# yc-huang/bsdb

Measured on AMD Instinct MI355X. Metric: index-build keys/s (device-resident), 13B x 13-byte keys; % HBM roofline, higher is better.
Workload: dtype u64

## Files before the change

### bsdb_amd/csrc/bsdb_capi.hip

```cpp
#include <hip/hip_runtime.h>

#include <dlfcn.h>
#include <sched.h>
#include <fcntl.h>
#include <sys/mman.h>
#include <sys/stat.h>
#include <unistd.h>

#include <algorithm>
#include <atomic>
#include <cerrno>
#include <functional>
#include <chrono>
#include <condition_variable>
#include <cmath>
#include <cstdio>
#include <cstdlib>
#include <cstring>
#include <memory>
#include <mutex>
#include <new>
#include <shared_mutex>
#include <string>
#include <thread>
#include <condition_variable>
#include <deque>
#include <vector>

#include "../../include/bsdb_mi355x.h"
#include "hash_kernels.hip"
#include "fused_kernels.hip"
#include "mph_kernels.hip"
#include "gov_kernels.hip"
#include "verify_kernels.hip"

using namespace bsdb;

struct FeedSlot {
    void *buf[8] = {};
    size_t cap[8] = {};
    hipEvent_t copied = nullptr, done = nullptr;
    bool used = false;
    std::vector<uint64_t> reb;
};

struct bsdb_ctx {
    int device = 0;
    hipStream_t stream = nullptr;
    int hist_mode = 0;
    int frontend = 0;
    int num_cus = 256;
    int d13_variant = 13;
    int d13_copies = 8;
    uint64_t chunk_keys = 0;
    uint64_t span_max = 0;
    int fused = -1;
    int pipe = -1;
    uint64_t pipe_chunks = 0;
    uint32_t pipe_cus = 0;
    hipStream_t p2_stream = nullptr;
    hipEvent_t pipe_ev[6] = {};
    void *fu_ring = nullptr;
    size_t fu_ring_bytes = 0;
    uint64_t fu_launches = 0;
    std::mutex mu;
    void *ids = nullptr;
    size_t ids_bytes = 0;
    uint32_t *cursor = nullptr;
    size_t cursor_bytes = 0;
    uint64_t *p2_pref = nullptr;
    size_t p2_pref_bytes = 0;
    uint32_t *overflow = nullptr;
    uint64_t *scan_part = nullptr;
    size_t scan_part_n = 0;
    FeedSlot feed[2];
    hipStream_t copy_stream = nullptr;
    void *d_out = nullptr;
    size_t d_out_bytes = 0;
    void *g_sorted = nullptr, *g_counts = nullptr, *g_cursor = nullptr, *g_scratch = nullptr, *g_status = nullptr;
    size_t g_sorted_bytes = 0, g_counts_bytes = 0, g_cursor_bytes = 0, g_scratch_bytes = 0, g_status_bytes = 0;
    void *g_big = nullptr, *g_slabs = nullptr;
    size_t g_big_bytes = 0, g_slabs_bytes = 0;
    void *g_pay = nullptr;
    size_t g_pay_bytes = 0;
    void *g_led = nullptr;
    size_t g_led_bytes = 0;
    void *g_mid = nullptr;
    size_t g_mid_bytes = 0;
    void *g_midscr = nullptr;
    size_t g_midscr_bytes = 0;
    hipStream_t big_stream = nullptr;
    hipEvent_t big_ev[2] = {nullptr, nullptr};
    bool verify = false;
    hipEvent_t last_ev = nullptr;
    hipStream_t last_stream = nullptr;
    void *comm = nullptr;
    int nranks = 1, rank = 0;
    std::mutex mph_mu;
    std::vector<bsdb_mph *> mphs;
    void *pack = nullptr;
    size_t pack_bytes = 0;
    bool profiling = false;
    struct Rec { hipEvent_t a, b; int kind; uint64_t keys; };
    std::vector<Rec> recs;
    std::vector<hipEvent_t> pool;
    hipEvent_t ev() {
        if (!pool.empty()) { hipEvent_t e = pool.back(); pool.pop_back(); return e; }
        hipEvent_t e = nullptr;
        (void)hipEventCreate(&e);
        return e;
    }
};

struct Ordered {
    bsdb_ctx *c;
    hipStream_t s;
    Ordered(bsdb_ctx *c_, hipStream_t s_) : c(c_), s(s_) {
        if (c->last_ev && c->last_stream != s) (void)hipStreamWaitEvent(s, c->last_ev, 0);
    }
    ~Ordered() {
        if (!c->last_ev && hipEventCreateWithFlags(&c->last_ev, hipEventDisableTiming) != hipSuccess) c->last_ev = nullptr;
        if (c->last_ev) (void)hipEventRecord(c->last_ev, s);
        c->last_stream = s;
    }
};

struct ProfScope {
    bsdb_ctx *c; hipStream_t s; int kind; uint64_t keys; hipEvent_t a = nullptr;
    ProfScope(bsdb_ctx *c_, hipStream_t s_, int k, uint64_t n) : c(c_), s(s_), kind(k), keys(n) {
        if (c->profiling) { a = c->ev(); (void)hipEventRecord(a, s); }
    }
    ~ProfScope() {
        if (!a) return;
        hipEvent_t b = c->ev();
        (void)hipEventRecord(b, s);
        c->recs.push_back({a, b, kind, keys});
    }
};

static void comm_destroy(bsdb_ctx *c);

namespace {

constexpr uint64_t DEFAULT_CHUNK_KEYS = 1ULL << 32;
constexpr uint64_t MAX_SPAN_LAUNCHES = 8;

int hip_fail(hipError_t e, const char *what, int line) {
    static const bool dbg = getenv("BSDB_DEBUG") != nullptr;
    if (dbg) fprintf(stderr, "[bsdb] line %d: %s -> %d (%s)\n", line, what, (int)e, hipGetErrorString(e));
    return BSDB_EIO;
}
#define HIP_OK(x)                                                   \
    do {                                                            \
        const hipError_t e_ = (x);                                  \
        if (e_ != hipSuccess) return hip_fail(e_, #x, __LINE__);    \
    } while (0)

template <class T>
hipError_t dmalloc(T **p, size_t bytes) {
    const hipError_t e = hipMalloc(reinterpret_cast<void **>(p), bytes);
    if (e != hipSuccess) {
        (void)hipGetLastError();
        *p = nullptr;
    }
    return e;
}

int grow(void **p, size_t *have, size_t need) {
    if (*have >= need) return BSDB_OK;
    if (*p) (void)hipFree(*p);
    *p = nullptr;
    *have = 0;
    const size_t roomy = need >= (1u << 20) ? need + need / 64 : need;
    if (roomy != need && dmalloc(p, roomy) == hipSuccess) {
        *have = roomy;
        return BSDB_OK;
    }
    if (dmalloc(p, need) != hipSuccess) return BSDB_ENOMEM;
    *have = need;
    return BSDB_OK;
}

constexpr size_t XFER_PIECE = 32ull << 20;

struct PinnedPool {
    std::mutex mu;
    std::vector<void *> free_list;
    void *take() {
        {
            std::lock_guard<std::mutex> g(mu);
            if (!free_list.empty()) {
                void *p = free_list.back();
                free_list.pop_back();
                return p;
            }
        }
        void *p = nullptr;
        if (hipHostMalloc(&p, XFER_PIECE, hipHostMallocDefault) == hipSuccess) return p;
        (void)hipGetLastError();
        return nullptr;
    }
    void give(void *p) {
        if (!p) return;
        std::lock_guard<std::mutex> g(mu);
        free_list.push_back(p);
    }
};
PinnedPool &pinned_pool() {
    static PinnedPool *pool = new PinnedPool();
    return *pool;
}

int file_reserve(int fd, uint64_t off, uint64_t len) {
    if (fd < 0 || !len) return 0;
    int r;
    do {
        r = fallocate(fd, 0, (off_t)off, (off_t)len);
    } while (r != 0 && errno == EINTR);
    if (r == 0) return 0;
    return errno == EOPNOTSUPP || errno == ENOSYS ? 1 : -1;
}

struct Populator {
    std::thread th;
    std::atomic<bool> stop{false};
    std::atomic<uint64_t> ready{0};
    int fd = -1;
    uint64_t file_off = 0;
    double seconds = 0;
    Populator() = default;
    Populator(const Populator &) = delete;
    Populator &operator=(const Populator &) = delete;
    ~Populator() { finish(); }
    void start(uint8_t *base, uint64_t bytes, int file_fd = -1, uint64_t base_off = 0) {
        fd = file_fd;
        file_off = base_off;
        if (!base || !bytes || getenv("BSDB_NO_PREFAULT")) return;
        th = std::thread([this, base, bytes] {
            const auto t0 = std::chrono::steady_clock::now();
            constexpr uint64_t STEP = 16ull << 20;
            constexpr int MADV_POPULATE_WRITE_ = 23;
            bool madv = true;
            for (uint64_t o = 0; o < bytes && !stop.load(std::memory_order_relaxed); o += STEP) {
                const uint64_t k = std::min(STEP, bytes - o);
                if (fd >= 0) {
                    if (file_reserve(fd, file_off + o, k) != 0) break;
                    ready.store(o + k, std::memory_order_release);
                }
                if (madv) {
                    if (madvise(base + o, k, MADV_POPULATE_WRITE_) == 0) continue;
                    if (errno != EINVAL) break;
                    madv = false;
                }
                for (uint64_t q = 0; q < k; q += 4096) (void)*(volatile const uint8_t *)(base + o + q);
            }
            seconds = std::chrono::duration<double>(std::chrono::steady_clock::now() - t0).count();
        });
    }
    bool ensure(uint64_t off, uint64_t len) {
        if (fd < 0 || off + len <= ready.load(std::memory_order_acquire)) return true;
        return file_reserve(fd, file_off + off, len) == 0;
    }
    void finish() {
        stop.store(true);
        if (th.joinable()) th.join();
    }
};

int copy_on_own_stream(int dev, void *dst, const void *src, size_t bytes, hipMemcpyKind kind) {
    if (bytes == 0) return BSDB_OK;
    hipStream_t s = nullptr;
    hipError_t e = hipSetDevice(dev);
    if (e == hipSuccess) e = hipStreamCreateWithFlags(&s, hipStreamNonBlocking);
    if (e == hipSuccess) e = hipMemcpyAsync(dst, src, bytes, kind, s);
    if (e == hipSuccess) e = hipStreamSynchronize(s);
    if (s) (void)hipStreamDestroy(s);
    return e == hipSuccess ? BSDB_OK : hip_fail(e, kind == hipMemcpyHostToDevice ? "H2D copy (own stream)" : "D2H copy (own stream)", __LINE__);
}
struct BounceSlots {
    std::mutex mu;
    std::condition_variable cv;
    int free_slots;
    BounceSlots() {
        const char *e = getenv("BSDB_BOUNCE_SLOTS");
        const int v = e ? atoi(e) : 16;
        free_slots = v > 0 ? v : 1;
    }
    void acquire() {
        std::unique_lock<std::mutex> g(mu);
        cv.wait(g, [this] { return free_slots > 0; });
        --free_slots;
    }
    void release() {
        {
            std::lock_guard<std::mutex> g(mu);
            ++free_slots;
        }
        cv.notify_one();
    }
};
static BounceSlots &bounce_slots() {
    static BounceSlots *b = new BounceSlots();
    return *b;
}
int h2d_bounce(hipStream_t s, void *dst, const void *src, size_t bytes) {
    if (bytes == 0) return BSDB_OK;
    bounce_slots().acquire();
    void *pin[2] = {pinned_pool().take(), pinned_pool().take()};
    if (!pin[0] || !pin[1]) {
        pinned_pool().give(pin[0]);
        pinned_pool().give(pin[1]);
        bounce_slots().release();
        hipError_t e = hipMemcpyAsync(dst, src, bytes, hipMemcpyHostToDevice, s);
        if (e == hipSuccess) e = hipStreamSynchronize(s);
        return e == hipSuccess ? BSDB_OK : hip_fail(e, "H2D copy (pageable fallback)", __LINE__);
    }
    hipEvent_t ev[2] = {nullptr, nullptr};
    int rc = BSDB_OK;
    for (int i = 0; i < 2 && !rc; ++i)
        if (hipEventCreateWithFlags(&ev[i], hipEventDisableTiming) != hipSuccess) rc = BSDB_EIO;
    bool pending[2] = {false, false};
    for (size_t o = 0, k = 0; o < bytes && !rc; o += XFER_PIECE, ++k) {
        const int i = (int)(k & 1);
        const size_t len = std::min(XFER_PIECE, bytes - o);
        if (pending[i] && hipEventSynchronize(ev[i]) != hipSuccess) rc = BSDB_EIO;
        if (rc) break;
        memcpy(pin[i], (const uint8_t *)src + o, len);
        if (hipMemcpyAsync((uint8_t *)dst + o, pin[i], len, hipMemcpyHostToDevice, s) != hipSuccess ||
            hipEventRecord(ev[i], s) != hipSuccess)
            rc = BSDB_EIO;
        pending[i] = true;
    }
    if (hipStreamSynchronize(s) != hipSuccess && !rc) rc = BSDB_EIO;
    for (int i = 0; i < 2; ++i) {
        pinned_pool().give(pin[i]);
        if (ev[i]) (void)hipEventDestroy(ev[i]);
    }
    bounce_slots().release();
    return rc;
}

int d2h_pageable(int dev, void *dst, const void *src, size_t bytes) {
    return copy_on_own_stream(dev, dst, src, bytes, hipMemcpyDeviceToHost);
}
int h2d_pageable(int dev, void *dst, const void *src, size_t bytes) {
    return copy_on_own_stream(dev, dst, src, bytes, hipMemcpyHostToDevice);
}

hipStream_t pick(bsdb_ctx *, void *stream) { return (hipStream_t)stream; }

int launch_status() {
    const hipError_t e = hipGetLastError();
    return e == hipSuccess ? BSDB_OK : hip_fail(e, "kernel launch", 0);
}

int usable_cpus() {
    static const int n = [] {
        int c = (int)std::max(1u, std::thread::hardware_concurrency());
        cpu_set_t cs;
        if (sched_getaffinity(0, sizeof(cs), &cs) == 0) c = std::max(1, CPU_COUNT(&cs));
        if (FILE *f = fopen("/sys/fs/cgroup/cpu.max", "r")) {
            char q[32] = {0};
            unsigned long long per = 0;
            if (fscanf(f, "%31s %llu", q, &per) == 2 && strcmp(q, "max") != 0 && per > 0) {
                const unsigned long long quota = strtoull(q, nullptr, 10);
                if (quota > 0) c = std::min<int>(c, (int)std::max<unsigned long long>(1, (quota + per - 1) / per));
            }
            fclose(f);
        }
        return c;
    }();
    return n;
}

constexpr uint64_t MAX_TILES_PER_LAUNCH = (1ULL << 32) / P1_THREADS - 1;

template <int EPI>
void launch_pass1(const P1Args &a0, bool var, uint32_t key_len, uint64_t tiles, hipStream_t s, int frontend) {
    if (tiles > MAX_TILES_PER_LAUNCH) {
        for (uint64_t t0 = 0; t0 < tiles; t0 += MAX_TILES_PER_LAUNCH) {
            const uint64_t nt = std::min(MAX_TILES_PER_LAUNCH, tiles - t0);
            P1Args a = a0;
            const uint64_t k0 = t0 * P1_TILE;
            a.n = std::min<uint64_t>(a0.n - k0, nt * P1_TILE);
            if (var) {
                a.offsets = a0.offsets + k0;
            } else {
                a.keys = a0.keys + k0 * key_len;
                a.blob_bytes = a0.blob_bytes - k0 * key_len;
            }
            if (a.sig) a.sig = a0.sig + 2 * k0;
            launch_pass1<EPI>(a, var, key_len, nt, s, frontend);
        }
        return;
    }
    const P1Args &a = a0;
    const dim3 g((uint32_t)tiles), b(P1_THREADS);
    if (var && frontend == 2) {
        k_pass1<SRC_VAR, EPI, 1, 0><<<g, b, 0, s>>>(a);
    } else if (var) {
        k_pass1<SRC_VARSTAGED, EPI, 1, 0><<<g, b, 0, s>>>(a);
    } else if (key_len == 13 && frontend != 1) {
        k_pass1<SRC_DIRECT13, EPI, 4, 13><<<g, b, 0, s>>>(a);
    } else if (key_len == 13) {
        k_pass1<SRC_STAGED13, EPI, 4, 13><<<g, b, 0, s>>>(a);
    } else if (key_len >= 1 && key_len <= 13) {
        k_pass1<SRC_STAGED, EPI, 4, 0><<<g, b, 0, s>>>(a);
    } else if (key_len >= 14 && key_len <= 26) {
        k_pass1<SRC_STAGED, EPI, 2, 0><<<g, b, 0, s>>>(a);
    } else if (key_len >= 27 && key_len <= 52) {
        k_pass1<SRC_STAGED, EPI, 1, 0><<<g, b, 0, s>>>(a);
    } else {
        k_pass1<SRC_FIXED_DIRECT, EPI, 1, 0><<<g, b, 0, s>>>(a);
    }
}

struct PartPlan {
    uint32_t nparts;
    uint32_t bin_shift;
    uint32_t capb;
    uint32_t nmain;
    uint32_t ntail;
    uint32_t grid_d13;
    uint64_t cap;
    uint64_t cap_tail;
    size_t ids_elems() const { return (size_t)nparts * (nmain * cap + ntail * cap_tail); }
};

uint64_t round64(double x) { return ((uint64_t)x + 63) & ~63ULL; }

using D13Kernel = void (*)(P1Args, uint64_t);

struct Pass1Sel {
    D13Kernel k;
    int nt;
    uint64_t tile;
    bool binned;
    bool windowed;
    uint32_t bin_shift;
    uint32_t nparts;
    uint32_t capb;
};

bool binned_layout(Pass1Sel &sel, uint32_t maxp, uint32_t bin_ids, uint64_t m) {
    uint32_t shift = 0;
    while (shift <= (uint32_t)PART_SHIFT && ((m + (1ULL << shift) - 1) >> shift) > (uint64_t)maxp) ++shift;
    if (shift > (uint32_t)PART_SHIFT) return false;
    sel.bin_shift = shift;
    sel.nparts = (uint32_t)((m + (1ULL << shift) - 1) >> shift);
    sel.capb = std::min<uint32_t>((bin_ids / sel.nparts) & ~7u, (uint32_t)sel.tile + 8);
    return true;
}

Pass1Sel pass1_select(const bsdb_ctx *c, bool var, uint32_t key_len, bool seed0, uint64_t m) {
    const uint32_t nparts = (uint32_t)((m + PART_BUCKETS - 1) / PART_BUCKETS);
    const Pass1Sel none{nullptr, 0, 0, false, false, (uint32_t)PART_SHIFT, nparts, 0};
    const Pass1Sel sort{k_pass1_d13<512>, 512, 512 * P1_KEYS_PER_THREAD, false, true, (uint32_t)PART_SHIFT, nparts, 0};
    const bool sort_fits = nparts <= 1024;
    if (c->frontend != 0) return none;
    const bool k13 = !var && key_len == 13;
    const bool window = k13 || (!var && (key_len == 8 || key_len == 12 || key_len == 16) && !getenv("BSDB_NO_FIXED_WINDOW"));
    if (window) {
        if (k13 && c->d13_variant == 2) return sort_fits ? sort : none;
        D13Kernel k = key_len == 8    ? (seed0 ? k_pass1_d13e<0, true, 8> : k_pass1_d13e<0, false, 8>)
                      : key_len == 12 ? (seed0 ? k_pass1_d13e<0, true, 12> : k_pass1_d13e<0, false, 12>)
                      : key_len == 16 ? (seed0 ? k_pass1_d13e<0, true, 16> : k_pass1_d13e<0, false, 16>)
                      : c->d13_variant == 13 ? (seed0 ? k_pass1_d13e<13, true> : k_pass1_d13e<13>)
                                             : (seed0 ? k_pass1_d13e<0, true> : k_pass1_d13e<0>);
        Pass1Sel sel{k, D13E_NT, D13E_TILE, true, true, 0, 0, 0};
        if (binned_layout(sel, D13E_MAXP, D13E_BIN_IDS, m)) return sel;
        return k13 && sort_fits ? sort : none;
    }
    if (!var && (key_len == 0 || key_len > 32)) return none;
    D13Kernel k = var ? (seed0 ? k_pass1_vare<false, true> : k_pass1_vare<false>)
                      : (seed0 ? k_pass1_vare<true, true> : k_pass1_vare<true>);
    Pass1Sel sel{k, VARE_NT, VARE_TILE, true, false, 0, 0, 0};
    return binned_layout(sel, VARE_MAXP, VARE_BIN_IDS, m) ? sel : none;
}

PartPlan plan_partitions(const bsdb_ctx *c, uint64_t chunk, uint64_t m, const Pass1Sel &sel) {
    PartPlan p{};
    const bool d13 = sel.k != nullptr, binned = sel.binned;
    p.bin_shift = sel.bin_shift;
    p.nparts = sel.nparts;
    p.capb = sel.capb;
    const double frac = std::min(1.0, (double)(1ULL << p.bin_shift) / (double)m);
    p.nmain = binned ? (uint32_t)c->d13_copies : NCOPY;
    const double e = (double)chunk * frac / p.nmain;
    p.cap = round64(e * 1.02 + 8.0 * std::sqrt(e) + 2 * P1_TILE + 64);
    p.ntail = 0;
    p.cap_tail = 0;
    if (d13) {
        int per_cu = 0;
        if (hipOccupancyMaxActiveBlocksPerMultiprocessor(&per_cu, sel.k, sel.nt, 0) != hipSuccess || per_cu < 1) per_cu = 1;
        per_cu = std::min(per_cu, 2048 / sel.nt);
        const uint64_t tiles = (chunk + sel.tile - 1) / sel.tile;
        p.grid_d13 = (uint32_t)std::min<uint64_t>(tiles, (uint64_t)c->num_cus * per_cu);
        if (const char *v = getenv("BSDB_D13_GRID")) p.grid_d13 = (uint32_t)std::max<int64_t>(1, std::min<int64_t>(p.grid_d13, atoll(v)));
        if (binned) {
            const double tiles_per_copy = (double)tiles / p.nmain + 1;
            p.cap = round64(e * 1.02 + 8.0 * std::sqrt(e) + 7.0 * tiles_per_copy + 2 * P1_TILE + 64);
        }
        p.ntail = NCOPY;
        p.cap_tail = round64(std::max<uint64_t>(P1_TILE, sel.tile) + 64);
    }
    return p;
}

constexpr uint64_t FU_MIN_SUPER = 4;

int fused13_impl(bsdb_ctx *c, const uint8_t *keys, uint64_t blob_bytes, uint64_t n, uint64_t seed, uint64_t m,
                 uint32_t *counts, hipStream_t s, uint64_t *done) {
    *done = 0;
    const uint64_t per = (uint64_t)FU_OWNERS * FU_TILE;
    if (c->num_cus != FU_OWNERS || m == 0 || m > (uint64_t)FU_OWNERS * (FU_TCAP - 2)) return BSDB_OK;
    if (blob_bytes < 3) return BSDB_OK;
    const uint64_t nsuper = std::min(n / per, (blob_bytes - 3) / 13 / per);
    if (nsuper < FU_MIN_SUPER) return BSDB_OK;
    if (n / m > 16384) return BSDB_OK;
    static int per_cu = -1;
    if (per_cu < 0 && hipOccupancyMaxActiveBlocksPerMultiprocessor(&per_cu, k_hist13_fused<true>, FU_NT, 0) != hipSuccess)
        per_cu = 0;
    if (per_cu < 1) return BSDB_OK;
    const size_t sync_bytes = FU_SYNC_U64 * sizeof(uint64_t);
    const size_t ring_bytes = (size_t)FU_SLOTS * FU_SLOT_BYTES;
    int rc = grow(&c->fu_ring, &c->fu_ring_bytes, ring_bytes + sync_bytes);
    if (rc) return rc;
    FusedArgs fa{};
    fa.keys = keys;
    fa.nsuper = nsuper;
    fa.seed = seed;
    fa.mult = (uint32_t)(2 * m);
    fa.m = (uint32_t)m;
    fa.ring = (uint8_t *)c->fu_ring;
    fa.sync = (uint64_t *)((uint8_t *)c->fu_ring + ring_bytes);
    fa.overflow = c->overflow;
    fa.counts = counts;
    HIP_OK(hipMemsetAsync(fa.sync, 0, sync_bytes, s));
    HIP_OK(hipMemsetAsync(c->overflow, 0, sizeof(uint32_t), s));
    ++c->fu_launches;
    {
        ProfScope ps(c, s, 0, nsuper * per);
        if (seed == 0 && !getenv("BSDB_NO_SEED0"))
            k_hist13_fused<true><<<FU_OWNERS, FU_NT, 0, s>>>(fa);
        else
            k_hist13_fused<false><<<FU_OWNERS, FU_NT, 0, s>>>(fa);
    }
    P1Args af{};
    af.keys = keys;
    af.blob_bytes = blob_bytes;
    af.key_len = 13;
    af.n = nsuper * per;
    af.seed = seed;
    af.multiplier = 2 * m;
    af.counts = counts;
    af.overflow = c->overflow;
    k_overflow_fallback<SRC_FIXED_DIRECT, 0><<<1024, P1_THREADS, 0, s>>>(af);
    if ((rc = launch_status())) return rc;
    *done = nsuper * per;
    return BSDB_OK;
}

bool pipe_wanted(const bsdb_ctx *c) { return c->pipe == 1; }

uint32_t pipe_p2_cus(const bsdb_ctx *c) {
    const uint32_t k = c->pipe_cus ? c->pipe_cus : (uint32_t)c->num_cus / 8;
    return std::max<uint32_t>(1, std::min<uint32_t>(k, (uint32_t)c->num_cus / 2));
}

bool fused_wanted(const bsdb_ctx *c) {
    if (c->hist_mode == 3) return true;
    if (c->hist_mode != 0) return false;
    if (c->fused >= 0) return c->fused == 1;
    return false;
}

int histogram_impl(bsdb_ctx *c, const uint8_t *keys, const uint64_t *offsets, uint64_t blob_bytes,
                   uint32_t key_len, uint64_t n, uint64_t seed, uint64_t m, uint32_t *counts,
                   hipStream_t s) {
    if (n == 0) return BSDB_OK;
    const bool var = offsets != nullptr;
    if (!var && key_len == 13 && fused_wanted(c)) {
        uint64_t done = 0;
        const int rc = fused13_impl(c, keys, blob_bytes, n, seed, m, counts, s, &done);
        if (rc) return rc;
        if (done) return histogram_impl(c, keys + done * 13, nullptr, blob_bytes - done * 13, 13, n - done, seed, m,
                                        counts, s);
    }
    P1Args a{};
    a.keys = keys;
    a.offsets = offsets;
    a.blob_bytes = blob_bytes;
    a.key_len = key_len;
    a.seed = seed;
    a.multiplier = 2 * m;
    a.counts = counts;
    const uint32_t nparts = (uint32_t)((m + PART_BUCKETS - 1) / PART_BUCKETS);
    const bool atomic_mode = c->hist_mode == 2 || nparts > (uint32_t)MAX_PARTS;
    if (atomic_mode) {
        a.n = n;
        ProfScope ps(c, s, 0, n);
        launch_pass1<EPI_ATOMIC>(a, var, key_len, (n + P1_TILE - 1) / P1_TILE, s, c->frontend);
        return launch_status();
    }
    uint64_t chunk = c->chunk_keys ? c->chunk_keys : DEFAULT_CHUNK_KEYS;
    chunk = std::max<uint64_t>(P1_TILE, chunk / P1_TILE * P1_TILE);
    chunk = std::min<uint64_t>(chunk, (n + P1_TILE - 1) / P1_TILE * P1_TILE);
    const Pass1Sel sel = pass1_select(c, var, key_len, seed == 0 && !getenv("BSDB_NO_SEED0"), m);
    const bool d13 = sel.k != nullptr;
    const bool pipe_pl = pipe_wanted(c) && sel.windowed && sel.binned;
    if (pipe_pl && !c->chunk_keys) {
        const uint64_t nch = c->pipe_chunks ? c->pipe_chunks : 8;
        chunk = std::max<uint64_t>(sel.tile, ((n + nch - 1) / nch + sel.tile - 1) / sel.tile * sel.tile);
    }
    auto whole_tiles = [&](uint64_t ch) {
        return d13 && !pipe_pl && ch < n && ch >= sel.tile ? ch / sel.tile * sel.tile : ch;
    };
    chunk = whole_tiles(chunk);
    PartPlan pp = plan_partitions(c, chunk, m, sel);
    size_t free_b = 0, total_b = 0;
    if (hipMemGetInfo(&free_b, &total_b) != hipSuccess) free_b = 0;
    const size_t budget = (free_b + c->ids_bytes) / 2 / (pipe_pl ? 2 : 1);
    while (chunk > 2 * P1_TILE && (pp.ids_elems() * sizeof(uint16_t) > budget ||
                                   (uint64_t)pp.nparts * pp.cap >= (1ULL << 32))) {
        chunk = whole_tiles(std::max<uint64_t>(P1_TILE, chunk / 2 / P1_TILE * P1_TILE));
        pp = plan_partitions(c, chunk, m, sel);
    }
    const size_t set_elems = (size_t)pp.nparts * pp.nmain * pp.cap;
    const size_t tail_elems = (size_t)pp.nparts * pp.ntail * pp.cap_tail;
    uint64_t J = 1;
    if (!pipe_pl && n > chunk && (!d13 || chunk % sel.tile == 0)) {
        const uint64_t jmax = c->span_max ? c->span_max : MAX_SPAN_LAUNCHES;
        J = std::min<uint64_t>({(n + chunk - 1) / chunk, jmax, MAX_SPAN_LAUNCHES});
        while (J > 1 && (J * set_elems + tail_elems) * sizeof(uint16_t) > budget) --J;
    }
    const uint32_t R = (uint32_t)J * pp.nmain + pp.ntail;
    const bool pipe = pipe_pl && n > chunk;
    const int nbuf = pipe ? 2 : 1;
    const size_t ids_per_buf = J * set_elems + tail_elems, cur_per_buf = (size_t)pp.nparts * R;
    int rc = grow(&c->ids, &c->ids_bytes, nbuf * ids_per_buf * sizeof(uint16_t));
    if (rc) return rc;
    rc = grow((void **)&c->cursor, &c->cursor_bytes,
              (nbuf * cur_per_buf + P1_SCRATCH_WG + (size_t)P1_SCRATCH_MAXWG * 1024) * sizeof(uint32_t));
    if (rc) return rc;
    rc = grow((void **)&c->p2_pref, &c->p2_pref_bytes, nbuf * (cur_per_buf + 1) * sizeof(uint64_t));
    if (rc) return rc;
    hipStream_t s2 = s;
    if (pipe) {
        if (!c->p2_stream && hipStreamCreateWithFlags(&c->p2_stream, hipStreamNonBlocking) != hipSuccess) return BSDB_EIO;
        for (auto &e : c->pipe_ev)
            if (!e && hipEventCreateWithFlags(&e, hipEventDisableTiming) != hipSuccess) return BSDB_EIO;
        s2 = c->p2_stream;
        HIP_OK(hipEventRecord(c->pipe_ev[4], s));
        HIP_OK(hipStreamWaitEvent(s2, c->pipe_ev[4], 0));
    }
    const uint32_t p2_cus = pipe ? pipe_p2_cus(c) : 0;
    a.scratch = c->cursor + nbuf * cur_per_buf;
    a.cap = pp.cap;
    a.nparts = pp.nparts;
    a.nregions = pp.nmain;
    a.region0 = 0;
    a.ncopy = pp.nmain;
    a.bin_shift = pp.bin_shift;
    a.capb = pp.capb;
    P2Layout L0{};
    L0.cap = pp.cap;
    L0.cap_tail = pp.cap_tail;
    L0.nparts = pp.nparts;
    L0.nmain = pp.nmain;
    L0.ntail = pp.ntail;
    L0.bshift = PART_SHIFT - pp.bin_shift;
    L0.num_buckets = m;
    L0.counts = counts;
    uint64_t i = 0;
    for (uint64_t s0 = 0; s0 < n; s0 += J * chunk) {
        const uint64_t ns = std::min(J * chunk, n - s0), jn = (ns + chunk - 1) / chunk;
        const bool last = s0 + ns >= n;
        const uint32_t b = pipe ? (uint32_t)(i & 1) : 0;
        P1Args as = a;
        as.ids = (uint16_t *)c->ids + b * ids_per_buf;
        as.cursor = c->cursor + b * cur_per_buf;
        as.overflow = c->overflow + 4 * b;
        uint64_t *pref = c->p2_pref + b * (cur_per_buf + 1);
        uint16_t *const tail_ids = as.ids + jn * set_elems;
        uint32_t *const tail_cur = as.cursor + jn * pp.nmain * pp.nparts;
        P2Layout L = L0;
        L.ids = as.ids;
        L.cursor = as.cursor;
        L.overflow = as.overflow;
        L.nmain = (uint32_t)jn * pp.nmain;
        const size_t cur_span = (size_t)pp.nparts * (L.nmain + L.ntail);
        as.n = ns;
        if (var) {
            as.offsets = offsets + s0;
        } else {
            as.keys = keys + s0 * key_len;
            as.blob_bytes = pipe ? blob_bytes - s0 * key_len : ns * key_len;
        }
        if (pipe && i >= 2) HIP_OK(hipStreamWaitEvent(s, c->pipe_ev[2 + b], 0));
        HIP_OK(hipMemsetAsync(as.cursor, 0, sizeof(uint32_t) * cur_span, s));
        HIP_OK(hipMemsetAsync(as.overflow, 0, sizeof(uint32_t), s));
        for (uint64_t j = 0; j < jn; ++j, ++i) {
            const uint64_t k0 = s0 + j * chunk, nk = std::min(chunk, n - k0);
            const bool first = k0 == 0, last_of_span = j + 1 == jn;
            P1Args ac = as;
            ac.ids = as.ids + j * set_elems;
            ac.cursor = as.cursor + j * pp.nmain * pp.nparts;
            ac.n = nk;
            if (var) {
                ac.offsets = offsets + k0;
            } else {
                ac.keys = keys + k0 * key_len;
                const bool to_end = pipe || !last_of_span;
                ac.blob_bytes = to_end ? blob_bytes - k0 * key_len : nk * key_len;
            }
            ProfScope ps(c, s, 0, nk);
            const uint64_t tiles = (nk + P1_TILE - 1) / P1_TILE;
            auto tail = [&](uint64_t done) {
                P1Args at = ac;
                at.n = nk - done;
                at.ids = tail_ids;
                at.cursor = tail_cur;
                at.cap = pp.cap_tail;
                at.nregions = pp.ntail;
                if (var) {
                    at.offsets = ac.offsets + done;
                    k_pass1<SRC_VAR, EPI_PARTITION, 1, 0><<<(uint32_t)((at.n + P1_TILE - 1) / P1_TILE), P1_THREADS, 0, s>>>(at);
                } else {
                    at.keys = ac.keys + done * key_len;
                    at.blob_bytes = at.n * key_len;
                    launch_pass1<EPI_PARTITION>(at, false, key_len, (at.n + P1_TILE - 1) / P1_TILE, s, 0);
                }
            };
            if (d13 && !sel.windowed) {
                const uint64_t nfast = nk / sel.tile;
                if (nfast) {
                    const uint32_t grid = (uint32_t)std::min<uint64_t>(nfast, pp.grid_d13);
                    sel.k<<<grid, sel.nt, 0, s>>>(ac, nfast);
                }
                if (nfast * sel.tile < nk) tail(nfast * sel.tile);
            } else if (d13) {
                const uint64_t dtile = sel.tile, over = 16 - key_len;
                uint64_t nfast = 0;
                if (ac.blob_bytes >= over) nfast = std::min(nk / dtile, ((ac.blob_bytes - over) / key_len) / dtile);
                if (nfast) {
                    uint32_t grid = (uint32_t)std::min<uint64_t>(nfast, pp.grid_d13);
                    if (pipe && !first) grid = std::max<uint32_t>(1, std::min<uint32_t>(grid, (uint32_t)c->num_cus - p2_cus));
                    sel.k<<<grid, sel.nt, 0, s>>>(ac, nfast);
                }
                if (nfast * dtile < nk) tail(nfast * dtile);
            } else {
                launch_pass1<EPI_PARTITION>(ac, var, key_len, tiles, s, c->frontend);
            }
        }
        if (pipe) {
            HIP_OK(hipEventRecord(c->pipe_ev[b], s));
            HIP_OK(hipStreamWaitEvent(s2, c->pipe_ev[b], 0));
        }
        {
            ProfScope ps(c, s2, 1, ns);
            k_pass2_plan<<<1, SCAN_THREADS, 0, s2>>>(L, pref);
            const uint32_t g2 = pipe && !last ? p2_cus : (uint32_t)c->num_cus;
            k_pass2b<<<g2, P2_THREADS, 0, s2>>>(L, pref);
        }
        if (var) {
            k_overflow_fallback<SRC_VAR, 0><<<1024, P1_THREADS, 0, s2>>>(as);
        } else {
            k_overflow_fallback<SRC_FIXED_DIRECT, 0><<<1024, P1_THREADS, 0, s2>>>(as);
        }
        if (pipe) HIP_OK(hipEventRecord(c->pipe_ev[2 + b], s2));
        if ((rc = launch_status())) return rc;
    }
    if (pipe) {
        HIP_OK(hipEventRecord(c->pipe_ev[5], s2));
        HIP_OK(hipStreamWaitEvent(s, c->pipe_ev[5], 0));
    }
    return BSDB_OK;
}

int hash_impl(bsdb_ctx *c, const uint8_t *keys, const uint64_t *offsets, uint64_t blob_bytes, uint32_t key_len,
              uint64_t n, uint64_t seed, uint64_t *sig, hipStream_t s) {
    if (n == 0) return BSDB_OK;
    P1Args a{};
    a.keys = keys;
    a.offsets = offsets;
    a.blob_bytes = blob_bytes;
    a.key_len = key_len;
    a.n = n;
    a.seed = seed;
    a.sig = sig;
    launch_pass1<EPI_SIG>(a, offsets != nullptr, key_len, (n + P1_TILE - 1) / P1_TILE, s, c->frontend);
    return launch_status();
}

bool aligned16(const void *p) { return ((uintptr_t)p & 15) == 0; }

bool bad_key_len(uint32_t key_len) { return key_len == 0 || key_len > 255; }

}

extern "C" {

int bsdb_abi_version(void) { return BSDB_ABI_VERSION; }

const char *bsdb_strerror(int code) {
    switch (code) {
        case BSDB_OK: return "ok";
        case BSDB_EINVAL: return "invalid argument";
        case BSDB_ENOMEM: return "device out of memory";
        case BSDB_EIO: return "HIP runtime error";
        case BSDB_ENODEV: return "no such HIP device";
        case BSDB_EDUP: return "duplicate key signature";
        case BSDB_ESEEDS: return "exhausted local seeds";
        case BSDB_E2BIG: return "bucket too large for the device solver";
        case BSDB_ECOMM: return "RCCL unavailable or collective failed";
        case BSDB_EFILE: return "file open/read/write failed";
        case BSDB_EVERIFY: return "built MPHF failed the bijection check";
        default: return "unknown error";
    }
}

uint64_t bsdb_num_buckets(uint64_t n) { return n / BUCKET_SIZE + 1; }

int bsdb_open(int device, bsdb_ctx **out) {
    if (!out) return BSDB_EINVAL;
    *out = nullptr;
    int ndev = 0;
    if (hipGetDeviceCount(&ndev) != hipSuccess || device < 0 || device >= ndev) return BSDB_ENODEV;
    bsdb_ctx *c = new (std::nothrow) bsdb_ctx();
    if (!c) return BSDB_ENOMEM;
    c->device = device;
    if (const char *v = std::getenv("BSDB_D13_VARIANT")) c->d13_variant = std::atoi(v);
    if (const char *v = std::getenv("BSDB_SPAN_MAX")) c->span_max = std::strtoull(v, nullptr, 10);
    if (const char *v = std::getenv("BSDB_FUSED")) c->fused = std::atoi(v) ? 1 : 0;
    if (const char *v = std::getenv("BSDB_PIPE")) c->pipe = std::atoi(v) ? 1 : 0;
    if (const char *v = std::getenv("BSDB_PIPE_CHUNKS")) c->pipe_chunks = std::strtoull(v, nullptr, 10);
    if (const char *v = std::getenv("BSDB_PIPE_P2CUS")) c->pipe_cus = (uint32_t)std::atoi(v);
    if (const char *v = std::getenv("BSDB_D13_COPIES")) {
        const int k = std::atoi(v);
        c->d13_copies = (k == 16 || k == 32 || k == 64) ? k : 8;
    }
    int cus = 0;
    if (hipDeviceGetAttribute(&cus, hipDeviceAttributeMultiprocessorCount, device) == hipSuccess && cus > 0)
        c->num_cus = cus;
    if (hipSetDevice(device) != hipSuccess || hipStreamCreateWithFlags(&c->stream, hipStreamNonBlocking) != hipSuccess) {
        delete c;
        return BSDB_EIO;
    }
    if (dmalloc(&c->overflow, sizeof(uint32_t) * 8) != hipSuccess ||
        hipMemset(c->overflow, 0, sizeof(uint32_t) * 8) != hipSuccess) {
        bsdb_close(c);
        return BSDB_ENOMEM;
    }
    *out = c;
    return BSDB_OK;
}

static void mph_detach_all(bsdb_ctx *c);

static void release_workspace(bsdb_ctx *c) {
    for (void **p : {&c->ids, &c->d_out, &c->g_sorted, &c->g_pay, &c->g_scratch, &c->g_led, &c->g_mid, &c->g_slabs,
                     &c->g_big, &c->pack, &c->g_midscr}) {
        (void)hipFree(*p);
        *p = nullptr;
    }
    c->ids_bytes = c->d_out_bytes = c->g_sorted_bytes = c->g_pay_bytes = c->g_scratch_bytes = c->g_led_bytes =
        c->g_mid_bytes = c->g_slabs_bytes = c->g_big_bytes = c->pack_bytes = c->g_midscr_bytes = 0;
    for (auto &f : c->feed) {
        if (f.used) (void)hipEventSynchronize(f.done);
        for (int i = 0; i < 8; ++i) {
            (void)hipFree(f.buf[i]);
            f.buf[i] = nullptr;
            f.cap[i] = 0;
        }
        f.used = false;
    }
}

int bsdb_release_workspace(bsdb_ctx *c) {
    if (!c) return BSDB_EINVAL;
    std::lock_guard<std::mutex> g(c->mu);
    HIP_OK(hipSetDevice(c->device));
    HIP_OK(hipDeviceSynchronize());
    release_workspace(c);
    return BSDB_OK;
}

int bsdb_close(bsdb_ctx *c) {
    if (!c) return BSDB_EINVAL;
    (void)hipSetDevice(c->device);
    if (c->stream) (void)hipStreamSynchronize(c->stream);
    mph_detach_all(c);
    (void)hipFree(c->ids);
    (void)hipFree(c->cursor);
    (void)hipFree(c->p2_pref);
    (void)hipFree(c->fu_ring);
    if (c->p2_stream) (void)hipStreamSynchronize(c->p2_stream);
    for (hipEvent_t e : c->pipe_ev)
        if (e) (void)hipEventDestroy(e);
    if (c->p2_stream) (void)hipStreamDestroy(c->p2_stream);
    (void)hipFree(c->overflow);
    (void)hipFree(c->scan_part);
    if (c->copy_stream) (void)hipStreamSynchronize(c->copy_stream);
    for (auto &f : c->feed) {
        for (void *p : f.buf) (void)hipFree(p);
        if (f.copied) (void)hipEventDestroy(f.copied);
        if (f.done) (void)hipEventDestroy(f.done);
    }
    if (c->copy_stream) (void)hipStreamDestroy(c->copy_stream);
    if (c->big_stream) (void)hipStreamSynchronize(c->big_stream);
    for (hipEvent_t e : c->big_ev)
        if (e) (void)hipEventDestroy(e);
    if (c->big_stream) (void)hipStreamDestroy(c->big_stream);
    (void)hipFree(c->d_out);
    (void)hipFree(c->g_sorted);
    (void)hipFree(c->g_counts);
    (void)hipFree(c->g_cursor);
    (void)hipFree(c->g_scratch);
    (void)hipFree(c->g_status);
    (void)hipFree(c->g_big);
    (void)hipFree(c->g_pay);
    (void)hipFree(c->g_led);
    (void)hipFree(c->g_mid);
    (void)hipFree(c->g_slabs);
    (void)hipFree(c->g_midscr);
    (void)hipFree(c->pack);
    comm_destroy(c);
    if (c->last_ev) (void)hipEventDestroy(c->last_ev);
    for (auto &r : c->recs) { (void)hipEventDestroy(r.a); (void)hipEventDestroy(r.b); }
    for (auto e : c->pool) (void)hipEventDestroy(e);
    if (c->stream) (void)hipStreamDestroy(c->stream);
    delete c;
    return BSDB_OK;
}

int bsdb_set_histogram_mode(bsdb_ctx *c, int mode) {
    if (!c || mode < 0 || mode > 3) return BSDB_EINVAL;
    std::lock_guard<std::mutex> g(c->mu);
    c->hist_mode = mode;
    return BSDB_OK;
}

int bsdb_set_frontend(bsdb_ctx *c, int frontend) {
    if (!c || frontend < 0 || frontend > 2) return BSDB_EINVAL;
    std::lock_guard<std::mutex> g(c->mu);
    c->frontend = frontend;
    return BSDB_OK;
}

int bsdb_fallback_count(bsdb_ctx *c, uint64_t *out) {
    if (!c || !out) return BSDB_EINVAL;
    std::lock_guard<std::mutex> g(c->mu);
    HIP_OK(hipSetDevice(c->device));
    HIP_OK(hipDeviceSynchronize());
    uint32_t v[8] = {};
    HIP_OK(hipMemcpy(v, c->overflow, sizeof(v), hipMemcpyDeviceToHost));
    *out = (uint64_t)v[2] + v[6];
    return BSDB_OK;
}

int bsdb_set_pipeline(bsdb_ctx *c, int mode, uint64_t chunks, uint32_t p2_cus) {
    if (!c || mode < -1 || mode > 1) return BSDB_EINVAL;
    std::lock_guard<std::mutex> g(c->mu);
    c->pipe = mode;
    c->pipe_chunks = chunks;
    c->pipe_cus = p2_cus;
    return BSDB_OK;
}

int bsdb_fused_status(bsdb_ctx *c, uint64_t *launches, uint64_t *timeouts) {
    if (!c || !launches || !timeouts) return BSDB_EINVAL;
    std::lock_guard<std::mutex> g(c->mu);
    HIP_OK(hipSetDevice(c->device));
    HIP_OK(hipDeviceSynchronize());
    uint32_t v = 0;
    HIP_OK(hipMemcpy(&v, c->overflow + 3, sizeof(v), hipMemcpyDeviceToHost));
    *launches = c->fu_launches;
    *timeouts = v;
    return BSDB_OK;
}

int bsdb_set_chunk_keys(bsdb_ctx *c, uint64_t chunk_keys) {
    if (!c) return BSDB_EINVAL;
    std::lock_guard<std::mutex> g(c->mu);
    c->chunk_keys = chunk_keys;
    return BSDB_OK;
}

int bsdb_dev_hash_fixed(bsdb_ctx *c, const uint8_t *d_keys, uint32_t key_len, uint64_t n, uint64_t seed,
                        uint64_t *d_sig, void *stream) {
    if (!c || bad_key_len(key_len) || (n && (!d_keys || !d_sig)) || !aligned16(d_keys) || !aligned16(d_sig))
        return BSDB_EINVAL;
    std::lock_guard<std::mutex> g(c->mu);
    HIP_OK(hipSetDevice(c->device));
    return hash_impl(c, d_keys, nullptr, n * key_len, key_len, n, seed, d_sig, pick(c, stream));
}

int bsdb_dev_hash_var(bsdb_ctx *c, const uint8_t *d_blob, uint64_t blob_bytes, const uint64_t *d_off, uint64_t n,
                      uint64_t seed, uint64_t *d_sig, void *stream) {
    if (!c || (n && (!d_blob || !d_off || !d_sig)) || !aligned16(d_sig)) return BSDB_EINVAL;
    std::lock_guard<std::mutex> g(c->mu);
    HIP_OK(hipSetDevice(c->device));
    return hash_impl(c, d_blob, d_off, blob_bytes, 0, n, seed, d_sig, pick(c, stream));
}

int bsdb_dev_histogram_fixed(bsdb_ctx *c, const uint8_t *d_keys, uint32_t key_len, uint64_t n, uint64_t seed,
                             uint64_t m, uint32_t *d_counts, void *stream) {
    if (!c || bad_key_len(key_len) || m == 0 || m > 0x7FFFFFFFULL || (n && (!d_keys || !d_counts)) || !aligned16(d_keys))
        return BSDB_EINVAL;
    std::lock_guard<std::mutex> g(c->mu);
// ... 737 lines not shown
```

Measured before the change: 309.7 billion.

## Share one region set across all span launches instead of per-launch copies

Launches within a span now append into a single shared set of partition regions, with capacity sized for the whole span, instead of each launch getting its own set of copies. The fixed cap of eight launches per span is removed, so a span can cover all of n when memory allows, and J is halved before the chunk size is reduced. The intent is fewer phase-2 passes and fewer region fragments (fewer cursors and less padding), so the build needs fewer pass-2 rounds. In exchange, cursor counts and capacities must fit in 32 bits across the whole span, and the windowed padding estimate now scales with grid size times the number of launches.

```diff
diff --git a/bsdb_amd/csrc/bsdb_capi.hip b/bsdb_amd/csrc/bsdb_capi.hip
--- a/bsdb_amd/csrc/bsdb_capi.hip
+++ b/bsdb_amd/csrc/bsdb_capi.hip
@@ -143,7 +143,6 @@
 namespace {
 
 constexpr uint64_t DEFAULT_CHUNK_KEYS = 1ULL << 32;
-constexpr uint64_t MAX_SPAN_LAUNCHES = 8;
 
 int hip_fail(hipError_t e, const char *what, int line) {
     static const bool dbg = getenv("BSDB_DEBUG") != nullptr;
@@ -478,7 +477,8 @@
     return binned_layout(sel, VARE_MAXP, VARE_BIN_IDS, m) ? sel : none;
 }
 
-PartPlan plan_partitions(const bsdb_ctx *c, uint64_t chunk, uint64_t m, const Pass1Sel &sel) {
+PartPlan plan_partitions(const bsdb_ctx *c, uint64_t span, uint64_t launch, uint64_t m, const Pass1Sel &sel,
+                         uint64_t *keys_per_copy = nullptr) {
     PartPlan p{};
     const bool d13 = sel.k != nullptr, binned = sel.binned;
     p.bin_shift = sel.bin_shift;
@@ -486,24 +486,33 @@
     p.capb = sel.capb;
     const double frac = std::min(1.0, (double)(1ULL << p.bin_shift) / (double)m);
     p.nmain = binned ? (uint32_t)c->d13_copies : NCOPY;
-    const double e = (double)chunk * frac / p.nmain;
-    p.cap = round64(e * 1.02 + 8.0 * std::sqrt(e) + 2 * P1_TILE + 64);
+    launch = std::min(launch, span);
+    const uint64_t tile = d13 ? sel.tile : (uint64_t)P1_TILE;
+    const uint64_t full = span / launch, rest = span % launch;
+    const uint64_t launches = full + (rest ? 1 : 0);
+    auto copy_tiles = [&](uint64_t keys) { return ((keys + tile - 1) / tile + p.nmain - 1) / p.nmain; };
+    const uint64_t tiles_per_copy = full * copy_tiles(launch) + copy_tiles(rest);
+    const uint64_t kpc = std::min(span, tiles_per_copy * tile);
+    if (keys_per_copy) *keys_per_copy = kpc;
+    const double e = (double)kpc * frac;
+    double pads = 0;
     p.ntail = 0;
     p.cap_tail = 0;
     if (d13) {
         int per_cu = 0;
         if (hipOccupancyMaxActiveBlocksPerMultiprocessor(&per_cu, sel.k, sel.nt, 0) != hipSuccess || per_cu < 1) per_cu = 1;
         per_cu = std::min(per_cu, 2048 / sel.nt);
-        const uint64_t tiles = (chunk + sel.tile - 1) / sel.tile;
+        const uint64_t tiles = (launch + sel.tile - 1) / sel.tile;
         p.grid_d13 = (uint32_t)std::min<uint64_t>(tiles, (uint64_t)c->num_cus * per_cu);
         if (const char *v = getenv("BSDB_D13_GRID")) p.grid_d13 = (uint32_t)std::max<int64_t>(1, std::min<int64_t>(p.grid_d13, atoll(v)));
-        if (binned) {
-            const double tiles_per_copy = (double)tiles / p.nmain + 1;
-            p.cap = round64(e * 1.02 + 8.0 * std::sqrt(e) + 7.0 * tiles_per_copy + 2 * P1_TILE + 64);
-        }
+        if (binned && sel.windowed)
+            pads = 7.0 * (p.grid_d13 / p.nmain + 1) * (double)launches;
+        else if (binned)
+            pads = 7.0 * (double)tiles_per_copy;
         p.ntail = NCOPY;
         p.cap_tail = round64(std::max<uint64_t>(P1_TILE, sel.tile) + 64);
     }
+    p.cap = round64(e * 1.02 + 8.0 * std::sqrt(e) + pads + 2 * P1_TILE + 64);
     return p;
 }
 
@@ -617,27 +626,32 @@
         return d13 && !pipe_pl && ch < n && ch >= sel.tile ? ch / sel.tile * sel.tile : ch;
     };
     chunk = whole_tiles(chunk);
-    PartPlan pp = plan_partitions(c, chunk, m, sel);
+    uint64_t J = 1;
+    if (!pipe_pl && n > chunk && (!d13 || chunk % sel.tile == 0)) {
+        J = (n + chunk - 1) / chunk;
+        if (c->span_max) J = std::min<uint64_t>(J, c->span_max);
+    }
     size_t free_b = 0, total_b = 0;
     if (hipMemGetInfo(&free_b, &total_b) != hipSuccess) free_b = 0;
     const size_t budget = (free_b + c->ids_bytes) / 2 / (pipe_pl ? 2 : 1);
-    while (chunk > 2 * P1_TILE && (pp.ids_elems() * sizeof(uint16_t) > budget ||
-                                   (uint64_t)pp.nparts * pp.cap >= (1ULL << 32))) {
-        chunk = whole_tiles(std::max<uint64_t>(P1_TILE, chunk / 2 / P1_TILE * P1_TILE));
-        pp = plan_partitions(c, chunk, m, sel);
+    uint64_t kpc = 0;
+    PartPlan pp = plan_partitions(c, std::min(n, J * chunk), chunk, m, sel, &kpc);
+    while (pp.ids_elems() * sizeof(uint16_t) > budget || (uint64_t)pp.nparts * pp.cap >= (1ULL << 32) ||
+           kpc >= (1ULL << 32)) {
+        if (J > 1)
+            J = (J + 1) / 2;
+        else if (chunk > 2 * P1_TILE)
+            chunk = whole_tiles(std::max<uint64_t>(P1_TILE, chunk / 2 / P1_TILE * P1_TILE));
+        else
+            break;
+        pp = plan_partitions(c, std::min(n, J * chunk), chunk, m, sel, &kpc);
     }
     const size_t set_elems = (size_t)pp.nparts * pp.nmain * pp.cap;
     const size_t tail_elems = (size_t)pp.nparts * pp.ntail * pp.cap_tail;
-    uint64_t J = 1;
-    if (!pipe_pl && n > chunk && (!d13 || chunk % sel.tile == 0)) {
-        const uint64_t jmax = c->span_max ? c->span_max : MAX_SPAN_LAUNCHES;
-        J = std::min<uint64_t>({(n + chunk - 1) / chunk, jmax, MAX_SPAN_LAUNCHES});
-        while (J > 1 && (J * set_elems + tail_elems) * sizeof(uint16_t) > budget) --J;
-    }
-    const uint32_t R = (uint32_t)J * pp.nmain + pp.ntail;
+    const uint32_t R = pp.nmain + pp.ntail;
     const bool pipe = pipe_pl && n > chunk;
     const int nbuf = pipe ? 2 : 1;
-    const size_t ids_per_buf = J * set_elems + tail_elems, cur_per_buf = (size_t)pp.nparts * R;
+    const size_t ids_per_buf = set_elems + tail_elems, cur_per_buf = (size_t)pp.nparts * R;
     int rc = grow(&c->ids, &c->ids_bytes, nbuf * ids_per_buf * sizeof(uint16_t));
     if (rc) return rc;
     rc = grow((void **)&c->cursor, &c->cursor_bytes,
@@ -682,14 +696,12 @@
         as.cursor = c->cursor + b * cur_per_buf;
         as.overflow = c->overflow + 4 * b;
         uint64_t *pref = c->p2_pref + b * (cur_per_buf + 1);
-        uint16_t *const tail_ids = as.ids + jn * set_elems;
-        uint32_t *const tail_cur = as.cursor + jn * pp.nmain * pp.nparts;
+        uint16_t *const tail_ids = as.ids + set_elems;
+        uint32_t *const tail_cur = as.cursor + pp.nmain * pp.nparts;
         P2Layout L = L0;
         L.ids = as.ids;
         L.cursor = as.cursor;
         L.overflow = as.overflow;
-        L.nmain = (uint32_t)jn * pp.nmain;
-        const size_t cur_span = (size_t)pp.nparts * (L.nmain + L.ntail);
         as.n = ns;
         if (var) {
             as.offsets = offsets + s0;
@@ -698,14 +710,12 @@
             as.blob_bytes = pipe ? blob_bytes - s0 * key_len : ns * key_len;
         }
         if (pipe && i >= 2) HIP_OK(hipStreamWaitEvent(s, c->pipe_ev[2 + b], 0));
-        HIP_OK(hipMemsetAsync(as.cursor, 0, sizeof(uint32_t) * cur_span, s));
+        HIP_OK(hipMemsetAsync(as.cursor, 0, sizeof(uint32_t) * cur_per_buf, s));
         HIP_OK(hipMemsetAsync(as.overflow, 0, sizeof(uint32_t), s));
         for (uint64_t j = 0; j < jn; ++j, ++i) {
             const uint64_t k0 = s0 + j * chunk, nk = std::min(chunk, n - k0);
             const bool first = k0 == 0, last_of_span = j + 1 == jn;
             P1Args ac = as;
-            ac.ids = as.ids + j * set_elems;
-            ac.cursor = as.cursor + j * pp.nmain * pp.nparts;
             ac.n = nk;
             if (var) {
                 ac.offsets = offsets + k0;
```

Result: faster. 315.4 billion (median of 6 runs) (+1.8%).
